# tsnuk/trade-AId-multimodal-transformer

Measured on AMD Instinct MI355X. Metric: training tokens/sec/GPU, 4-modality 1M-row synthetic, at 1/2/4/8 MI355X, higher is better.
Workload: dtype bf16; 1 GPU; C1: 4-modality 1M-row synthetic, d256 L6 T256 (BASELINE configs[1]); model=multimodal-transformer, global_batch=64, seq_len=256, n_embd=256, n_head=8, n_layer=6, modalities=4, parallelism=dp1

## Files before the change

### include/mmt.h

```cpp
#ifndef MMT_H_
#define MMT_H_
#include <stdint.h>

#ifdef __cplusplus
extern "C" {
#endif

#define MMT_MAX_MODALITIES 8

enum mmt_status {
  MMT_OK = 0,
  MMT_ERR_INVALID = -1,
  MMT_ERR_UNSUPPORTED = -2,
  MMT_ERR_HIP = -3,
  MMT_ERR_STATE = -4
};

typedef struct mmt_config {
  int32_t num_modalities;
  int32_t n_embd;
  int32_t n_head;
  int32_t n_layer;
  int32_t block_size;
  int32_t vocab_sizes[MMT_MAX_MODALITIES];
// ... 114 lines not shown
                   const int32_t* vocab, uint32_t* mt_state, const uint32_t* words, int64_t nwords, void* scratch,
                   int64_t scratch_bytes, int32_t* status);
int mmt_attn_set_ring(int v);
int mmt_attn_set_mask_g(int g);
int mmt_gemm_set_t2(int v);

int mmt_gemm_set_variant(int variant);
int mmt_op_gemm(void* stream, int32_t a_kc, int32_t b_kc, int32_t epi, int32_t splits, int32_t M, int32_t N,
                int32_t K, const void* A, int32_t lda, const void* B, int32_t ldb, const float* bias,
                const void* aux, int32_t ldaux, const float* resid, int32_t ldres, float* o32, int32_t ldc,
                void* o16, int32_t ldo16, float alpha);
int mmt_op_gemm_qkv(void* stream, int32_t M, int32_t N, int32_t K, const void* A, int32_t lda, const void* B,
                    int32_t ldb, const float* bias, void* h1, int32_t ldh1, const float* w2, int32_t hh, void* out,
                    int32_t ld_out);
int mmt_op_gemm_wgrad(void* stream, int32_t M, int32_t N, int32_t K, const void* A, int32_t lda, const void* B,
                      int32_t ldb, float* out, int32_t ldc, float alpha, void* slab, int64_t slab_bytes);
int mmt_op_mlp2(void* stream, int32_t M, int32_t C, const void* x, int32_t ldx, const void* w0, int32_t ldw0,
                const float* b0, const void* w2, int32_t ldw2, const float* b2, void* h, int32_t ldh, const float* resid,
                float* out, void* out16, uint32_t drop_key, uint32_t drop_thr, float drop_scale, const float* lnf_gamma,
                const float* lnf_beta, void* lnf_y, float* lnf_mean, float* lnf_rstd);
int mmt_op_mlp2_bwd(void* stream, int32_t M, int32_t C, const void* dy, int32_t lddy, const void* w2, int32_t ldw2,
                    const void* h, int32_t ldh, float alpha, const void* w0, int32_t ldw0, void* dh, int32_t lddh,
                    float* db0, void* dx);
int mmt_op_layernorm_fwd(void* stream, int32_t R, int32_t C, const float* x, const float* gamma, const float* beta,
                         void* y16, float* mean, float* rstd);
int mmt_op_layernorm_bwd(void* stream, int32_t R, int32_t C, const float* x, const float* gamma, const float* mean,
                         const float* rstd, const float* dy, float* dx, void* dx16, float* dgamma, float* dbeta);
int mmt_op_gemm_ln_bwd(void* stream, int32_t M, int32_t N, int32_t K, const void* A, int32_t lda, const void* B,
                       int32_t ldb, float alpha, const float* x, const float* gamma, const float* mean,
                       const float* rstd, float* dx, void* dx16, float* dgamma, float* dbeta, float* dsum,
                       uint32_t drop_key, uint32_t drop_thr, float drop_scale);
int mmt_op_attention_fwd(void* stream, int32_t B, int32_t T, int32_t H, int32_t hs, int32_t nstreams,
                         const void* q, int32_t q_ld, const void* const* k, const void* const* v, int32_t kv_ld,
                         int32_t kv_hstride, void* o, int32_t o_ld, void* const* oj, float* const* lse);
int mmt_op_attention_bwd(void* stream, int32_t B, int32_t T, int32_t H, int32_t hs, int32_t nstreams,
                         const void* q, int32_t q_ld, const void* const* k, const void* const* v, int32_t kv_ld,
                         int32_t kv_hstride, const void* o, int32_t o_ld, const void* const* oj,
                         const float* const* lse, const void* dout, int32_t dout_ld, float* const* dvec, void* dq,
                         int32_t dq_ld, void* const* dk, void* const* dv, int32_t dkv_ld, int32_t dkv_hstride);
int mmt_op_attention_bwd_ws(void* stream, int32_t B, int32_t T, int32_t H, int32_t hs, int32_t nstreams,
                            const void* q, int32_t q_ld, const void* const* k, const void* const* v, int32_t kv_ld,
                            int32_t kv_hstride, const void* o, int32_t o_ld, const void* const* oj,
                            const float* const* lse, const void* dout, int32_t dout_ld, float* const* dvec, void* dq,
                            int32_t dq_ld, void* const* dk, void* const* dv, int32_t dkv_ld, int32_t dkv_hstride,
                            float* dq32, int32_t dq32_ld);
int mmt_op_attention_fwd_h1(void* stream, int32_t B, int32_t T, int32_t H, const void* h1, int32_t ld_h1,
// ... 2 lines not shown
                            const float* w2, const void* o, int32_t o_ld, const float* lse, const void* dout,
                            int32_t dout_ld, void* dh1, float* dw2, float* db1);
int mmt_op_qkv2_fwd(void* stream, int32_t R, int32_t nblk, int32_t hs, const void* h1, int32_t ld_h1,
                    const float* w2, void* out, int32_t ld_out);
int mmt_op_qkv2_bwd(void* stream, int32_t R, int32_t nblk, int32_t hs, const void* h1, int32_t ld_h1,
                    const float* w2, const void* dout, int32_t ld_out, void* dh1, float* dw2);
int mmt_op_colsum(void* stream, int32_t R, int32_t N, const void* x, int32_t ld, float* out, float alpha);
int mmt_op_ordered_sum(void* stream, int32_t nparts, int32_t n, const float* parts, int64_t ld, float* dst);
int mmt_op_cross_entropy(void* stream, int32_t R, int32_t V, const float* logits, const int64_t* tgt,
                         void* dlogits, int32_t ld_d, float* loss);
int mmt_op_embedding_fwd(void* stream, int32_t B, int32_t T, int32_t C, int32_t V, const int64_t* idx,
                         const float* tok, const float* pos, float* x);
int mmt_op_embedding_bwd(void* stream, int32_t B, int32_t T, int32_t C, int32_t V, const int64_t* idx,
                         const float* dx, float* dtok, float* dpos);
int mmt_op_embedding_bwd_ws(void* stream, int32_t B, int32_t T, int32_t C, int32_t V, const int64_t* idx,
                            const float* dx, float* dtok, float* dpos, float* scratch);
int mmt_emb_set_sort(int on);
int mmt_qkv2_set_coal(int on);
int mmt_set_relu_bits(int on);
int mmt_set_drop_copy_fuse(int on);
int mmt_set_attn_qkv2(int on);
int mmt_set_attn_qkv_onchip(int bits);
int mmt_mlp2_set_bm(int bm);

int mmt_op_mx_quant(void* stream, int32_t rows, int32_t cols, const float* src, int32_t ld_src, void* dst8,
                    int32_t ld8, void* s8, int32_t lds8);
int mmt_op_gemm_f8(void* stream, int32_t epi, int32_t M, int32_t N, int32_t K, const void* A8, int32_t lda,
                   const void* sa, int32_t lds_a, const void* B8, int32_t ldb, const void* sb, int32_t lds_b,
                   const float* bias, const float* resid, int32_t ldres, float* o32, int32_t ldc, void* o16,
                   int32_t ldo16, void* o8, int32_t ld8, void* s8, int32_t lds8);
int mmt_op_layernorm_fwd_f8(void* stream, int32_t R, int32_t C, const float* x, const float* gamma, const float* beta,
                            void* y16, float* mean, float* rstd, void* y8, int32_t ld8, void* s8, int32_t lds8);

#ifdef __cplusplus
}
#endif
#endif
```

### trade-aid-multimodal-transformer_amd/csrc/mmt_engine.hip

```cpp
#include <hip/hip_runtime.h>

#include <algorithm>
#include <cmath>
#include <cstdio>
#include <cstdlib>
#include <cstring>
#include <string>
#include <vector>

#include "mmt.h"
#include "mmt_common.h"
#include "mmt_kernels.h"

namespace {

constexpr int MAXM = MMT_MAX_MODALITIES;

inline int64_t rup(int64_t x, int64_t a) { return (x + a - 1) / a * a; }
inline int r8(int x) { return (int)rup(x < 1 ? 1 : x, 8); }

struct Mat {
  int64_t off = -1;
  int rows = 0, cols = 0;
  int64_t pk = 0;
// ... 63 lines not shown

}

static int g_relu_bits = mmt_env_int("MMT_RELU_BITS", 0);
extern "C" int mmt_set_relu_bits(int on) {
  const int old = g_relu_bits;
  g_relu_bits = on;
  return old;
}
static int g_drop_copy_fuse = mmt_env_int("MMT_DROP_COPY_FUSE", 1);
extern "C" int mmt_set_drop_copy_fuse(int on) {
  const int old = g_drop_copy_fuse;
  g_drop_copy_fuse = on;
  return old;
}

static int g_attn_qkv2 = mmt_env_int("MMT_ATTN_QKV2", 1);
extern "C" int mmt_set_attn_qkv2(int on) {
  const int old = g_attn_qkv2;
  g_attn_qkv2 = on;
  return old;
}

static int g_attn_qkv_onchip = mmt_env_int("MMT_ATTN_QKV_ONCHIP", 3) & 3;
extern "C" int mmt_set_attn_qkv_onchip(int bits) {
  const int old = g_attn_qkv_onchip;
  g_attn_qkv_onchip = bits & 3;
  return old;
}

struct mmt_ctx {
  mmt_config cfg;
  int M, C, H, L, T, hs, hh;
  int V[MAXM];
  bool any_cross = false;
  int ncross = 0;
  std::vector<TensorInfo> tensors;
  std::vector<LM> lm;
  PostM post[MAXM];
  int64_t pos_off = 0;
  int64_t nparams = 0, nactive = 0;
  int64_t emb_begin = 0, emb_end = 0, post_begin = 0, post_end = 0;
  std::vector<int64_t> layer_begin, layer_end;
  std::vector<PackSeg> segs;
  std::vector<int> tasks;
  std::vector<MxSeg> mxsegs;
// ... 587 lines not shown
      Mlp2Batch& b = chunk[i / MMT_MLP2_GROUP];
      b.g1[b.count] = g1s[i];
      b.g2[b.count] = g2s[i];
      ++b.count;
    }
    for (int k = 0; k < nch; ++k)
      if (!(bwd ? mmt_mlp2_bwd_ok(chunk[k]) : mmt_mlp2_ok(chunk[k]))) return false;
    if (bwd)
      for (int k = 0; k < nch; ++k) det_arm(chunk[k]);
    const int id = probe_begin(what, s);
    for (int k = 0; k < nch; ++k) ok(bwd ? mmt_launch_mlp2_bwd(chunk[k], s) : mmt_launch_mlp2(chunk[k], s), what);
    if (id >= 0) {
      double fl = 0, by = 0;
      GemmBatch g1{}, g2{};
      g1.count = g2.count = n;
      for (int g = 0; g < n; ++g) { g1.p[g] = g1s[g]; g2.p[g] = g2s[g]; }
      gemm_cost(g1, bwd ? EPI_DTANH_BF16 : EPI_BIAS_TANH_BF16, &fl, &by);
      gemm_cost(g2, bwd ? EPI_STORE_BF16 : EPI_BIAS_RESID_F32, &fl, &by);
      for (int g = 0; g < n; ++g) by -= (double)g2s[g].M * g2s[g].K * 2.0;
      probe_end(id, s, fl, by);
    }
    return true;
  }
  bool gemm_resid_ln(const GemmBatch& b, const char* what) {
    if (rc != MMT_OK || !mmt_gemm_resid_ln_ok(b)) return false;
    const int id = probe_begin(what, s);
    ok(mmt_launch_gemm_resid_ln(b, s), what);
    if (id >= 0) {
      double fl = 0, by = 0;
      gemm_cost(b, EPI_BIAS_RESID_F32, &fl, &by);
      for (int g = 0; g < b.count; ++g)
        if (b.p[g].lnf_y) by += (double)b.p[g].M * b.p[g].N * 2.0 + b.p[g].M * 8.0;
      probe_end(id, s, fl, by);
    }
    return true;
  }
  int gemm_hint = 0;
  void gemm(const GemmBatch& b, bool akc, bool bkc, int epi, int splits, const char* what) {
    if (rc != MMT_OK) return;
    const int id = probe_begin(what, s);
    if (gemm_hint || det) {
      GemmBatch h = b;
      if (gemm_hint) h.tile_hint = gemm_hint;
      det_arm(h);
      ok(mmt_launch_gemm(h, akc, bkc, epi, splits, s), what);
    } else {
// ... 244 lines not shown
      ln2_done = fused && ln2_fuse;
      if (!fused) {
        for (int i = 0; i < M; ++i) g.p[i] = pg1[i];
        r.gemm(g, true, true, EPI_BIAS_TANH_BF16, 1, "proj0");
        for (int i = 0; i < M; ++i) { g.p[i] = pg2[i]; g.p[i].lnf_y = nullptr; }
        r.gemm(g, true, true, EPI_BIAS_RESID_F32, 1, "proj2");
      }
    }
    if (!ln2_done) {
      for (int i = 0; i < M; ++i) {
        lb.p[i].x = r.W<float>(a[i].x1); lb.p[i].gamma = r.P(x[i].ln2w); lb.p[i].beta = r.P(x[i].ln2b);
        lb.p[i].y = r.W<bf16_t>(a[i].c); lb.p[i].mean = r.W<float>(a[i].mean2); lb.p[i].rstd = r.W<float>(a[i].rstd2);
        ln8(lb.p[i], a[i].c8, a[i].cs8);
      }
      r.ok(mmt_launch_ln_fwd(lb, R, C, r.s), "ln2_fwd");
    }
    for (int i = 0; i < M; ++i) {
      g.p[i] = f8 ? gp_f8(r.W<uint8_t>(a[i].c8), C, r.W<uint8_t>(a[i].cs8), ldsC, w8, x[i].F0, R)
                  : gp_fwd(r.W<bf16_t>(a[i].c), C, wpk, x[i].F0, R);
      g.p[i].bias = r.P(x[i].bf0); g.p[i].o16 = r.W<bf16_t>(a[i].f); g.p[i].ldo16 = 4 * C;
      if (r.c->relu_bits) { g.p[i].mask8 = r.W<uint8_t>(a[i].fm); g.p[i].ldm8 = 4 * C / 8; }
      if (f8) { g.p[i].o8 = r.W<uint8_t>(a[i].f8); g.p[i].ld8 = 4 * C; g.p[i].s8 = r.W<uint8_t>(a[i].fs8); g.p[i].lds8 = ldsF; }
    }
    if (f8) r.gemm8(g, EPI_BIAS_RELU_BF16, "ffn0");
    else r.gemm(g, true, true, EPI_BIAS_RELU_BF16, 1, "ffn0");
    for (int i = 0; i < M; ++i) g.p[i].mask8 = nullptr;
    for (int i = 0; i < M; ++i) {
      g.p[i] = f8 ? gp_f8(r.W<uint8_t>(a[i].f8), 4 * C, r.W<uint8_t>(a[i].fs8), ldsF, w8, x[i].F2, R)
                  : gp_fwd(r.W<bf16_t>(a[i].f), 4 * C, wpk, x[i].F2, R);
      g.p[i].bias = r.P(x[i].bf2); g.p[i].resid = r.W<float>(a[i].x1); g.p[i].ldres = C;
      g.p[i].o32 = r.W<float>(a[i].x2); g.p[i].ldc = C;
      if (c->any_cross) { g.p[i].o16 = r.W<bf16_t>(a[i].x2h); g.p[i].ldo16 = C; }
      r.set_drop(g.p[i], l, i, DS_FFN);
    }
    bool lnc_done = false;
    if (fuse_fwd) {
      for (int i = 0; i < M; ++i) {
        GemmProblem& q = g.p[i];
        if (c->any_cross && x[i].cross) {
          q.lnf_gamma = r.P(x[i].lncw); q.lnf_beta = r.P(x[i].lncb); q.lnf_y = r.W<bf16_t>(a[i].d);
          q.lnf_mean = r.W<float>(a[i].meanc); q.lnf_rstd = r.W<float>(a[i].rstdc);
        } else if (l + 1 < c->L) {
          const LM& xn = c->lm[(size_t)(l + 1) * M + i];
          const ActLM& an = p.act[(size_t)(l + 1) * M + i];
          q.lnf_gamma = r.P(xn.ln1w); q.lnf_beta = r.P(xn.ln1b); q.lnf_y = r.W<bf16_t>(an.a);
          q.lnf_mean = r.W<float>(an.mean1); q.lnf_rstd = r.W<float>(an.rstd1);
        } else {
          q.lnf_gamma = r.P(c->post[i].lnw); q.lnf_beta = r.P(c->post[i].lnb); q.lnf_y = r.W<bf16_t>(p.lnf16[i]);
          q.lnf_mean = r.W<float>(p.meanf[i]); q.lnf_rstd = r.W<float>(p.rstdf[i]);
        }
      }
      if (r.gemm_resid_ln(g, "ffn2")) {
        for (int i = 0; i < M; ++i) {
          if (c->any_cross && x[i].cross) lnc_done = true;
          else if (l + 1 < c->L) ln1_done[i] = 1;
          else lnf_done[i] = 1;
        }
      } else {
        for (int i = 0; i < M; ++i) g.p[i].lnf_y = nullptr;
        r.gemm(g, true, true, EPI_BIAS_RESID_F32, 1, "ffn2");
      }
    } else if (f8) {
      r.gemm8(g, EPI_BIAS_RESID_F32, "ffn2");
    } else {
      r.gemm(g, true, true, EPI_BIAS_RESID_F32, 1, "ffn2");
    }
    for (int i = 0; i < M; ++i) g.p[i].lnf_y = nullptr;
    std::vector<const float*> xout(M);
    for (int i = 0; i < M; ++i) xout[i] = r.W<float>(a[i].x2);
    if (c->any_cross) {
      std::vector<int> cx;
      for (int i = 0; i < M; ++i) if (x[i].cross) cx.push_back(i);
      LnBatch lc{}; lc.count = (int)cx.size();
      GemmBatch gq{}; gq.count = (int)cx.size();
      for (size_t u = 0; u < cx.size(); ++u) {
        const int i = cx[u];
        lc.p[u].x = r.W<float>(a[i].x2); lc.p[u].gamma = r.P(x[i].lncw); lc.p[u].beta = r.P(x[i].lncb);
        lc.p[u].y = r.W<bf16_t>(a[i].d); lc.p[u].mean = r.W<float>(a[i].meanc); lc.p[u].rstd = r.W<float>(a[i].rstdc);
        ln8(lc.p[u], a[i].d8, a[i].ds8);
        gq.p[u] = f8 ? gp_f8(r.W<uint8_t>(a[i].d8), C, r.W<uint8_t>(a[i].ds8), ldsC, w8, x[i].Wq, R)
                     : gp_fwd(r.W<bf16_t>(a[i].d), C, wpk, x[i].Wq, R);
        gq.p[u].o16 = r.W<bf16_t>(a[i].qc); gq.p[u].ldo16 = C;
      }
      if (!lnc_done) r.ok(mmt_launch_ln_fwd(lc, R, C, r.s), "lnc_fwd");
      if (f8) r.gemm8(gq, EPI_STORE_BF16, "ca_q");
      else r.gemm(gq, true, true, EPI_STORE_BF16, 1, "ca_q");
      GemmBatch gk{}; gk.count = 0;
      for (int i : cx) {
// ... 1000 lines not shown
```

### trade-aid-multimodal-transformer_amd/csrc/mmt_gemm_dev.h

```cpp
#pragma once
#include "mmt_common.h"
#include "mmt_kernels.h"

#include <stdint.h>

template <int WM_, int WN_, int TM_, int TN_>
struct TileCfg {
  static constexpr int WM = WM_, WN = WN_, TM = TM_, TN = TN_;
  static constexpr int NW = WM * WN, NT = 64 * NW;
  static constexpr int BM = WM * TM * 32, BN = WN * TN * 32;
};
using TileS = TileCfg<2, 2, 2, 2>;
using TileL = TileCfg<2, 4, 4, 2>;
using TileW = TileCfg<1, 8, 4, 2>;

typedef __attribute__((address_space(3))) void lds_void;

__device__ __forceinline__ float* det_of(const GemmBatch& batch, int prob) {
  return batch.det.base ? batch.det.base + (int64_t)prob * batch.det.stride : nullptr;
}

template <int BK>
__device__ __forceinline__ int kc_swz(int chunk, int row) {
  return BK == 64 ? (chunk ^ ((row >> 1) & 7)) : (chunk ^ ((row >> 2) & 3));
// ... 152 lines not shown
  const int h = lane >> 5, r = lane & 31;
#pragma unroll
  for (int i = 0; i < TN; ++i)
#pragma unroll
    for (int j = 0; j < TM; ++j) {
      const int mf = wm * TM * 32 + 32 * j;
      if (mf / EPI_ROWS != pass) continue;
      const int ml = mf - pass * EPI_ROWS + r;
#pragma unroll
      for (int g = 0; g < 4; ++g) {
        const int nl = wn * TN * 32 + 32 * i + 8 * g + 4 * h;
        *reinterpret_cast<f32x4*>(ct + ml * CT + nl) =
            f32x4{acc[i][j][4 * g], acc[i][j][4 * g + 1], acc[i][j][4 * g + 2], acc[i][j][4 * g + 3]};
      }
    }
}
template <class TL, int EPI_ROWS>
__device__ __forceinline__ void stage_acc(f32x4 (&acc)[4][8], float* ct, int pass, int lane, int wave) {
  constexpr int CT = TL::BN + 4;
  const int wr = wave >> 2, wc = wave & 3;
#pragma unroll
  for (int mb = 0; mb < 8; ++mb) {
    const int mf = wr * 128 + 16 * mb;
    if (mf / EPI_ROWS != pass) continue;
    const int ml = mf - pass * EPI_ROWS + (lane & 15);
#pragma unroll
    for (int nb = 0; nb < 4; ++nb)
      *reinterpret_cast<f32x4*>(ct + ml * CT + wc * 64 + 16 * nb + 4 * (lane >> 4)) = acc[nb][mb];
  }
}

template <class TL, int EPI, int EPI_ROWS, bool PRE = false, class ACC>
__device__ __forceinline__ void epilogue_swap(const GemmProblem& P, ACC& acc, char* lds,
                                              float* o32, float alpha, int m0, int n0, int tid, int lane, int wave,
                                              float* det = nullptr) {
  constexpr int GBM = TL::BM, GBN = TL::BN, NW = TL::NW, NT = TL::NT, TM = TL::TM, TN = TL::TN;
  const int M = P.M, N = P.N;
  const int wm = wave / TL::WN, wn = wave % TL::WN;
  const int h = lane >> 5, r = lane & 31;
  constexpr int CT = GBN + 4;
  constexpr int TPR = GBN / 8;
  constexpr int RPI = NT / TPR;
  constexpr int IT = EPI_ROWS / RPI;
  float* ct = reinterpret_cast<float*>(lds);
  const int c8 = tid % TPR;
  const int rsub = tid / TPR;
// ... 381 lines not shown
```

### trade-aid-multimodal-transformer_amd/csrc/mmt_kernels.h

```cpp
#pragma once
#include <hip/hip_runtime.h>
#include <stdint.h>
#include "mmt_det.h"

#ifndef MMT_MAX_GROUP
#define MMT_MAX_GROUP 8
#endif
typedef uint16_t bf16_t;

enum MmtEpi {
  EPI_STORE_BF16 = 0,
  EPI_BIAS_TANH_BF16,
  EPI_BIAS_RELU_BF16,
  EPI_BIAS_RESID_F32,
  EPI_STORE_F32,
  EPI_DTANH_BF16,
  EPI_DRELU_BF16,
  EPI_ACC_F32,
  EPI_ATOMIC_F32,
  EPI_LN_BWD_F32,
  EPI_COUNT
};

struct GemmProblem {
// ... 45 lines not shown
  unsigned long long* stamps;
  DetScratch det;
};

hipError_t mmt_launch_gemm(const GemmBatch& b, bool a_kc, bool b_kc, int epi, int splits, hipStream_t s);
bool mmt_gemm_ln_bwd_ok(const GemmBatch& b);
bool mmt_gemm_resid_ln_ok(const GemmBatch& b);
hipError_t mmt_launch_gemm_resid_ln(const GemmBatch& b, hipStream_t s);
hipError_t mmt_launch_gemm_ln_bwd(const GemmBatch& b, hipStream_t s);
hipError_t mmt_launch_gemm_wgrad(const GemmBatch& b, float* slab, int64_t slab_bytes, hipStream_t s);

#define MMT_MLP2_GROUP 4
struct Mlp2Batch {
  GemmProblem g1[MMT_MLP2_GROUP];
  GemmProblem g2[MMT_MLP2_GROUP];
  int count;
  DetScratch det;
};
static_assert(sizeof(Mlp2Batch) <= 4096, "Mlp2Batch is a kernel argument");
bool mmt_mlp2_ok(const Mlp2Batch& b);
hipError_t mmt_launch_mlp2(const Mlp2Batch& b, hipStream_t s);
bool mmt_mlp2_bwd_ok(const Mlp2Batch& b);
hipError_t mmt_launch_mlp2_bwd(const Mlp2Batch& b, hipStream_t s);
hipError_t mmt_launch_gemm_f8(const GemmBatch& b, int epi, hipStream_t s);
bool mmt_gemm_wgrad_big(const GemmBatch& b);

struct LnProblem {
  const float* x;
  const float* gamma;
  const float* beta;
  bf16_t* y;
  float* mean;
  float* rstd;
  uint8_t* y8;
  uint8_t* s8;
  int ld8, lds8;
  const float* dy;
  float* dx;
  bf16_t* dx16;
  float* dgamma;
  float* dbeta;
  uint32_t drop_key, drop_thr;
  float drop_scale;
  float* dsum;
};
struct LnBatch {
// ... 166 lines not shown
```

### trade-aid-multimodal-transformer_amd/csrc/mmt_ops.hip

```cpp
#include <hip/hip_runtime.h>

#include "mmt.h"
#include "mmt_kernels.h"

static int st(hipError_t e) { return e == hipSuccess ? MMT_OK : MMT_ERR_HIP; }

extern "C" {

int mmt_op_gemm(void* stream, int32_t a_kc, int32_t b_kc, int32_t epi, int32_t splits, int32_t M, int32_t N,
                int32_t K, const void* A, int32_t lda, const void* B, int32_t ldb, const float* bias, const void* aux,
                int32_t ldaux, const float* resid, int32_t ldres, float* o32, int32_t ldc, void* o16, int32_t ldo16,
                float alpha) {
  if (epi < 0 || epi >= EPI_COUNT || M < 0 || N < 0 || K < 0) return MMT_ERR_INVALID;
  if ((lda & 7) || (ldb & 7)) return MMT_ERR_INVALID;
  GemmBatch b{};
  b.count = 1;
  GemmProblem& p = b.p[0];
  p.A = (const bf16_t*)A; p.lda = lda; p.B = (const bf16_t*)B; p.ldb = ldb; p.bias = bias;
  p.aux = (const bf16_t*)aux; p.ldaux = ldaux; p.resid = resid; p.ldres = ldres; p.o32 = o32; p.ldc = ldc;
  p.o16 = (bf16_t*)o16; p.ldo16 = ldo16; p.alpha = alpha; p.M = M; p.N = N; p.K = K;
  const hipError_t e = mmt_launch_gemm(b, a_kc != 0, b_kc != 0, epi, splits, (hipStream_t)stream);
  if (e == hipErrorInvalidValue) return MMT_ERR_UNSUPPORTED;
  return st(e);
}
// ... 25 lines not shown
  if (e == hipErrorInvalidValue) return MMT_ERR_UNSUPPORTED;
  return st(e);
}

int mmt_op_mlp2(void* stream, int32_t M, int32_t C, const void* x, int32_t ldx, const void* w0, int32_t ldw0,
                const float* b0, const void* w2, int32_t ldw2, const float* b2, void* h, int32_t ldh, const float* resid,
                float* out, void* out16, uint32_t drop_key, uint32_t drop_thr, float drop_scale, const float* lnf_gamma,
                const float* lnf_beta, void* lnf_y, float* lnf_mean, float* lnf_rstd) {
  if (M < 1 || C < 2) return MMT_ERR_INVALID;
  Mlp2Batch b{};
  b.count = 1;
  GemmProblem& p1 = b.g1[0];
  p1.A = (const bf16_t*)x; p1.lda = ldx; p1.B = (const bf16_t*)w0; p1.ldb = ldw0; p1.bias = b0;
  p1.o16 = (bf16_t*)h; p1.ldo16 = ldh; p1.alpha = 1.f; p1.M = M; p1.N = C / 2; p1.K = C;
  GemmProblem& p2 = b.g2[0];
  p2.A = (const bf16_t*)h; p2.lda = ldh; p2.B = (const bf16_t*)w2; p2.ldb = ldw2; p2.bias = b2;
  p2.resid = resid; p2.ldres = C; p2.o32 = out; p2.ldc = C; p2.o16 = (bf16_t*)out16; p2.ldo16 = C;
  p2.alpha = 1.f; p2.M = M; p2.N = C; p2.K = C / 2;
  p2.drop_key = drop_key; p2.drop_thr = drop_thr; p2.drop_scale = drop_scale;
  p2.lnf_gamma = lnf_gamma; p2.lnf_beta = lnf_beta; p2.lnf_y = (bf16_t*)lnf_y; p2.lnf_mean = lnf_mean;
  p2.lnf_rstd = lnf_rstd;
  if (!mmt_mlp2_ok(b)) return MMT_ERR_UNSUPPORTED;
  return st(mmt_launch_mlp2(b, (hipStream_t)stream));
}

int mmt_op_mlp2_bwd(void* stream, int32_t M, int32_t C, const void* dy, int32_t lddy, const void* w2, int32_t ldw2,
                    const void* h, int32_t ldh, float alpha, const void* w0, int32_t ldw0, void* dh, int32_t lddh,
                    float* db0, void* dx) {
  if (M < 1 || C < 2) return MMT_ERR_INVALID;
  Mlp2Batch b{};
  b.count = 1;
  GemmProblem& p1 = b.g1[0];
  p1.A = (const bf16_t*)dy; p1.lda = lddy; p1.B = (const bf16_t*)w2; p1.ldb = ldw2; p1.aux = (const bf16_t*)h;
  p1.ldaux = ldh; p1.o16 = (bf16_t*)dh; p1.ldo16 = lddh; p1.dbias = db0; p1.alpha = alpha; p1.M = M; p1.N = C / 2;
  p1.K = C;
  GemmProblem& p2 = b.g2[0];
  p2.A = (const bf16_t*)dh; p2.lda = lddh; p2.B = (const bf16_t*)w0; p2.ldb = ldw0; p2.o16 = (bf16_t*)dx; p2.ldo16 = C;
  p2.alpha = 1.f; p2.M = M; p2.N = C; p2.K = C / 2;
  if (!mmt_mlp2_bwd_ok(b)) return MMT_ERR_UNSUPPORTED;
  return st(mmt_launch_mlp2_bwd(b, (hipStream_t)stream));
}

int mmt_op_layernorm_fwd(void* stream, int32_t R, int32_t C, const float* x, const float* gamma, const float* beta,
                         void* y16, float* mean, float* rstd) {
  LnBatch b{};
  b.count = 1;
// ... 233 lines not shown
```

### trade-aid-multimodal-transformer_amd/mmt_build.py

```python
import concurrent.futures as cf
import os
import subprocess
import sys

HERE = os.path.dirname(os.path.abspath(__file__))
REPO = os.path.dirname(HERE)
CSRC = os.path.join(HERE, "csrc")
OBJ = os.path.join(CSRC, "build")
LIB = os.path.join(HERE, "libmmt_hip.so")
HIPCC = os.environ.get("HIPCC", "/opt/rocm/bin/hipcc")
SOURCES = ["mmt_gemm.hip", "mmt_gemm8.hip", "mmt_mlp2.hip", "mmt_attn.hip", "mmt_attn_oc.hip", "mmt_attn2.hip", "mmt_elem.hip", "mmt_stats.hip", "mmt_qkv2.hip", "mmt_engine.hip", "mmt_ops.hip", "mmt_batch.hip", "mmt_decode.hip"]
FLAGS = ["--offload-arch=gfx950", "-O3", "-std=c++17", "-fPIC", "-I" + os.path.join(REPO, "include"), "-I" + CSRC,
         "-Wall", "-Wno-unused-function", "-Wno-unused-variable", "-Wno-unused-result"]

VGPR_FORM = ["-mllvm", "-amdgpu-mfma-vgpr-form=1"]
FILE_FLAGS = {"mmt_attn.hip": ["-fno-slp-vectorize"] + VGPR_FORM, "mmt_attn_oc.hip": ["-fno-slp-vectorize"] + VGPR_FORM,
              "mmt_attn2.hip": ["-fno-slp-vectorize"],
              "mmt_qkv2.hip": VGPR_FORM}


def _deps_mtime():
    hdrs = [os.path.join(CSRC, f) for f in os.listdir(CSRC) if f.endswith(".h")]
    hdrs.append(os.path.join(REPO, "include", "mmt.h"))
    return max(os.path.getmtime(h) for h in hdrs)


def _compile(src, force):
    s = os.path.join(CSRC, src)
    o = os.path.join(OBJ, src.replace(".hip", ".o"))
    if not force and os.path.exists(o) and os.path.getmtime(o) >= max(os.path.getmtime(s), _deps_mtime()):
        return o
    cmd = [HIPCC] + FLAGS + FILE_FLAGS.get(src, []) + ["-c", s, "-o", o]
    r = subprocess.run(cmd, capture_output=True, text=True)
    if r.returncode != 0:
# ... 23 lines not shown
```

### trade-aid-multimodal-transformer_amd/mmt_lib.py

```python
import ctypes
import os

import torch

HERE = os.path.dirname(os.path.abspath(__file__))
LIB_PATH = os.environ.get("MMT_LIB_PATH") or os.path.join(HERE, "libmmt_hip.so")
MAX_MOD = 8

c_i32 = ctypes.c_int32
c_i64 = ctypes.c_int64
c_f32 = ctypes.c_float
c_vp = ctypes.c_void_p
c_cp = ctypes.c_char_p


class MmtConfig(ctypes.Structure):
    _fields_ = [
        ("num_modalities", c_i32),
        ("n_embd", c_i32),
        ("n_head", c_i32),
        ("n_layer", c_i32),
        ("block_size", c_i32),
        ("vocab_sizes", c_i32 * MAX_MOD),
        ("cross_attention", c_i32 * MAX_MOD),
# ... 91 lines not shown
    "mmt_set_deterministic": (c_i32, [c_vp, c_i32]),
    "mmt_get_deterministic": (c_i32, [c_vp]),
    "mmt_probe_count": (c_i32, [c_vp]),
    "mmt_probe_read_at": (c_i32, [c_vp, c_i32, ctypes.POINTER(ctypes.c_double), ctypes.POINTER(c_i64),
                                  ctypes.POINTER(ctypes.c_double), ctypes.POINTER(ctypes.c_double)]),
    "mmt_batch_jitter":(c_i32, [c_vp, c_vp, c_i64, c_i32, c_i32, ctypes.c_uint64, ctypes.c_uint64]),
    "mmt_batch_indices": (c_i32, [c_vp, c_i32, c_vp, c_vp, c_i32, c_i32, ctypes.c_uint64, ctypes.c_uint64, c_vp]),
    "mmt_batch_gather": (c_i32, [c_vp, c_i32, ctypes.POINTER(c_vp), c_vp, c_i32, c_i32, ctypes.POINTER(c_vp),
                                 ctypes.POINTER(c_vp)]),
    "mmt_exact_words_bytes": (c_i64, [c_i64]),
    "mmt_exact_walk_scratch_bytes": (c_i64, [c_i64, c_i64]),
    "mmt_exact_gen": (c_i32, [c_vp, c_vp, c_vp, c_i64]),
    "mmt_exact_walk": (c_i32, [c_vp, c_i32, ctypes.POINTER(c_vp), ctypes.POINTER(c_i64), ctypes.POINTER(c_i32),
                               ctypes.POINTER(c_i32), c_vp, c_vp, c_i64, c_vp, c_i64, c_vp]),
    "mmt_attn_set_ring": (c_i32, [ctypes.c_int]),
    "mmt_attn_set_mask_g": (c_i32, [ctypes.c_int]),
    "mmt_gemm_set_t2": (c_i32, [ctypes.c_int]),
    "mmt_emb_set_sort": (c_i32, [ctypes.c_int]),
    "mmt_set_relu_bits": (c_i32, [ctypes.c_int]),
    "mmt_set_drop_copy_fuse": (c_i32, [ctypes.c_int]),
    "mmt_set_attn_qkv2": (c_i32, [ctypes.c_int]),
    "mmt_set_attn_qkv_onchip": (c_i32, [ctypes.c_int]),
    "mmt_mlp2_set_bm": (c_i32, [ctypes.c_int]),
    "mmt_qkv2_set_coal": (c_i32, [ctypes.c_int]),
    "mmt_gemm_set_variant": (c_i32, [ctypes.c_int]),
    "mmt_op_gemm": (c_i32, [c_vp, c_i32, c_i32, c_i32, c_i32, c_i32, c_i32, c_i32, c_vp, c_i32, c_vp, c_i32, c_vp,
                            c_vp, c_i32, c_vp, c_i32, c_vp, c_i32, c_vp, c_i32, c_f32]),
    "mmt_op_gemm_qkv": (c_i32, [c_vp, c_i32, c_i32, c_i32, c_vp, c_i32, c_vp, c_i32, c_vp, c_vp, c_i32, c_vp, c_i32,
                                c_vp, c_i32]),
    "mmt_op_gemm_wgrad": (c_i32, [c_vp, c_i32, c_i32, c_i32, c_vp, c_i32, c_vp, c_i32, c_vp, c_i32, c_f32, c_vp, c_i64]),
    "mmt_op_gemm_ln_bwd": (c_i32, [c_vp, c_i32, c_i32, c_i32, c_vp, c_i32, c_vp, c_i32, c_f32, c_vp, c_vp, c_vp, c_vp,
                                   c_vp, c_vp, c_vp, c_vp, c_vp, ctypes.c_uint32, ctypes.c_uint32, c_f32]),
    "mmt_op_mlp2": (c_i32, [c_vp, c_i32, c_i32, c_vp, c_i32, c_vp, c_i32, c_vp, c_vp, c_i32, c_vp, c_vp, c_i32, c_vp,
                            c_vp, c_vp, ctypes.c_uint32, ctypes.c_uint32, c_f32, c_vp, c_vp, c_vp, c_vp, c_vp]),
    "mmt_op_mlp2_bwd": (c_i32, [c_vp, c_i32, c_i32, c_vp, c_i32, c_vp, c_i32, c_vp, c_i32, c_f32, c_vp, c_i32, c_vp,
                                c_i32, c_vp, c_vp]),
    "mmt_op_layernorm_fwd": (c_i32, [c_vp, c_i32, c_i32, c_vp, c_vp, c_vp, c_vp, c_vp, c_vp]),
    "mmt_op_layernorm_bwd": (c_i32, [c_vp, c_i32, c_i32, c_vp, c_vp, c_vp, c_vp, c_vp, c_vp, c_vp, c_vp, c_vp]),
    "mmt_op_attention_fwd": (c_i32, [c_vp, c_i32, c_i32, c_i32, c_i32, c_i32, c_vp, c_i32, ctypes.POINTER(c_vp),
                                     ctypes.POINTER(c_vp), c_i32, c_i32, c_vp, c_i32, ctypes.POINTER(c_vp),
                                     ctypes.POINTER(c_vp)]),
    "mmt_op_attention_bwd": (c_i32, [c_vp, c_i32, c_i32, c_i32, c_i32, c_i32, c_vp, c_i32, ctypes.POINTER(c_vp),
                                     ctypes.POINTER(c_vp), c_i32, c_i32, c_vp, c_i32, ctypes.POINTER(c_vp),
                                     ctypes.POINTER(c_vp), c_vp, c_i32, ctypes.POINTER(c_vp), c_vp, c_i32,
                                     ctypes.POINTER(c_vp), ctypes.POINTER(c_vp), c_i32, c_i32]),
    "mmt_op_attention_bwd_ws": (c_i32, [c_vp, c_i32, c_i32, c_i32, c_i32, c_i32, c_vp, c_i32, ctypes.POINTER(c_vp),
                                        ctypes.POINTER(c_vp), c_i32, c_i32, c_vp, c_i32, ctypes.POINTER(c_vp),
                                        ctypes.POINTER(c_vp), c_vp, c_i32, ctypes.POINTER(c_vp), c_vp, c_i32,
                                        ctypes.POINTER(c_vp), ctypes.POINTER(c_vp), c_i32, c_i32, c_vp, c_i32]),
    "mmt_op_attention_fwd_h1": (c_i32, [c_vp, c_i32, c_i32, c_i32, c_vp, c_i32, c_vp, c_vp, c_i32, c_vp]),
    "mmt_op_attention_bwd_h1": (c_i32, [c_vp, c_i32, c_i32, c_i32, c_vp, c_i32, c_vp, c_vp, c_i32, c_vp, c_vp, c_i32,
                                        c_vp, c_vp, c_vp]),
    "mmt_op_qkv2_fwd": (c_i32, [c_vp, c_i32, c_i32, c_i32, c_vp, c_i32, c_vp, c_vp, c_i32]),
    "mmt_op_qkv2_bwd": (c_i32, [c_vp, c_i32, c_i32, c_i32, c_vp, c_i32, c_vp, c_vp, c_i32, c_vp, c_vp]),
    "mmt_op_colsum": (c_i32, [c_vp, c_i32, c_i32, c_vp, c_i32, c_vp, c_f32]),
    "mmt_op_ordered_sum": (c_i32, [c_vp, c_i32, c_i32, c_vp, c_i64, c_vp]),
    "mmt_op_cross_entropy": (c_i32, [c_vp, c_i32, c_i32, c_vp, c_vp, c_vp, c_i32, c_vp]),
# ... 58 lines not shown
```

Measured before the change: 8.579 million tokens/s.

## Fuse FFN up-projection and down-projection into one on-chip forward kernel

```diff
diff --git a/include/mmt.h b/include/mmt.h
--- a/include/mmt.h
+++ b/include/mmt.h
@@ -160,6 +160,11 @@
 int mmt_op_mlp2_bwd(void* stream, int32_t M, int32_t C, const void* dy, int32_t lddy, const void* w2, int32_t ldw2,
                     const void* h, int32_t ldh, float alpha, const void* w0, int32_t ldw0, void* dh, int32_t lddh,
                     float* db0, void* dx);
+int mmt_op_ffn(void* stream, int32_t count, const int32_t* M, int32_t C, const void* const* x, int32_t ldx,
+               const void* w0, int32_t ldw0, const float* b0, const void* w2, int32_t ldw2, const float* b2,
+               void* const* h, int32_t ldh, const float* const* resid, float* const* out, void* const* out16,
+               uint32_t drop_key, uint32_t drop_thr, float drop_scale, const float* lnf_gamma, const float* lnf_beta,
+               void* const* lnf_y, float* const* lnf_mean, float* const* lnf_rstd);
 int mmt_op_layernorm_fwd(void* stream, int32_t R, int32_t C, const float* x, const float* gamma, const float* beta,
                          void* y16, float* mean, float* rstd);
 int mmt_op_layernorm_bwd(void* stream, int32_t R, int32_t C, const float* x, const float* gamma, const float* mean,
@@ -208,6 +213,7 @@
 int mmt_set_attn_qkv2(int on);
 int mmt_set_attn_qkv_onchip(int bits);
 int mmt_mlp2_set_bm(int bm);
+int mmt_set_ffn_fused(int on);
 
 int mmt_op_mx_quant(void* stream, int32_t rows, int32_t cols, const float* src, int32_t ld_src, void* dst8,
                     int32_t ld8, void* s8, int32_t lds8);
diff --git a/trade-aid-multimodal-transformer_amd/csrc/mmt_engine.hip b/trade-aid-multimodal-transformer_amd/csrc/mmt_engine.hip
--- a/trade-aid-multimodal-transformer_amd/csrc/mmt_engine.hip
+++ b/trade-aid-multimodal-transformer_amd/csrc/mmt_engine.hip
@@ -109,6 +109,12 @@
   return old;
 }
 
+static int g_ffn_fused = mmt_env_int("MMT_FFN_FUSED", 1);
+extern "C" int mmt_set_ffn_fused(int on) {
+  const int old = g_ffn_fused;
+  g_ffn_fused = on;
+  return old;
+}
 static int g_attn_qkv_onchip = mmt_env_int("MMT_ATTN_QKV_ONCHIP", 3) & 3;
 extern "C" int mmt_set_attn_qkv_onchip(int bits) {
   const int old = g_attn_qkv_onchip;
@@ -742,6 +748,32 @@
     }
     return true;
   }
+  bool ffn(const GemmProblem* g1s, const GemmProblem* g2s, int n, const char* what) {
+    if (rc != MMT_OK || n < 1) return false;
+    Mlp2Batch chunk[(MMT_MAX_GROUP + MMT_MLP2_GROUP - 1) / MMT_MLP2_GROUP] = {};
+    const int nch = (n + MMT_MLP2_GROUP - 1) / MMT_MLP2_GROUP;
+    for (int i = 0; i < n; ++i) {
+      Mlp2Batch& b = chunk[i / MMT_MLP2_GROUP];
+      b.g1[b.count] = g1s[i];
+      b.g2[b.count] = g2s[i];
+      ++b.count;
+    }
+    for (int k = 0; k < nch; ++k)
+      if (!mmt_ffn_ok(chunk[k])) return false;
+    const int id = probe_begin(what, s);
+    for (int k = 0; k < nch; ++k) ok(mmt_launch_ffn(chunk[k], s), what);
+    if (id >= 0) {
+      double fl = 0, by = 0;
+      GemmBatch g1{}, g2{};
+      g1.count = g2.count = n;
+      for (int g = 0; g < n; ++g) { g1.p[g] = g1s[g]; g2.p[g] = g2s[g]; }
+      gemm_cost(g1, EPI_BIAS_RELU_BF16, &fl, &by);
+      gemm_cost(g2, EPI_BIAS_RESID_F32, &fl, &by);
+      for (int g = 0; g < n; ++g) by -= (double)g2s[g].M * g2s[g].K * 2.0;
+      probe_end(id, s, fl, by);
+    }
+    return true;
+  }
   bool gemm_resid_ln(const GemmBatch& b, const char* what) {
     if (rc != MMT_OK || !mmt_gemm_resid_ln_ok(b)) return false;
     const int id = probe_begin(what, s);
@@ -1032,8 +1064,11 @@
       if (r.c->relu_bits) { g.p[i].mask8 = r.W<uint8_t>(a[i].fm); g.p[i].ldm8 = 4 * C / 8; }
       if (f8) { g.p[i].o8 = r.W<uint8_t>(a[i].f8); g.p[i].ld8 = 4 * C; g.p[i].s8 = r.W<uint8_t>(a[i].fs8); g.p[i].lds8 = ldsF; }
     }
-    if (f8) r.gemm8(g, EPI_BIAS_RELU_BF16, "ffn0");
-    else r.gemm(g, true, true, EPI_BIAS_RELU_BF16, 1, "ffn0");
+    const GemmBatch gf0 = g;
+    auto run_ffn0 = [&] {
+      if (f8) r.gemm8(gf0, EPI_BIAS_RELU_BF16, "ffn0");
+      else r.gemm(gf0, true, true, EPI_BIAS_RELU_BF16, 1, "ffn0");
+    };
     for (int i = 0; i < M; ++i) g.p[i].mask8 = nullptr;
     for (int i = 0; i < M; ++i) {
       g.p[i] = f8 ? gp_f8(r.W<uint8_t>(a[i].f8), 4 * C, r.W<uint8_t>(a[i].fs8), ldsF, w8, x[i].F2, R)
@@ -1060,7 +1095,11 @@
           q.lnf_mean = r.W<float>(p.meanf[i]); q.lnf_rstd = r.W<float>(p.rstdf[i]);
         }
       }
-      if (r.gemm_resid_ln(g, "ffn2")) {
+    }
+    const bool ffn_one = !f8 && !c->relu_bits && C == 256 && g_ffn_fused != 0 && r.ffn(gf0.p, g.p, M, "ffn");
+    if (!ffn_one) run_ffn0();
+    if (fuse_fwd) {
+      if (ffn_one || r.gemm_resid_ln(g, "ffn2")) {
         for (int i = 0; i < M; ++i) {
           if (c->any_cross && x[i].cross) lnc_done = true;
           else if (l + 1 < c->L) ln1_done[i] = 1;
@@ -1070,10 +1109,9 @@
         for (int i = 0; i < M; ++i) g.p[i].lnf_y = nullptr;
         r.gemm(g, true, true, EPI_BIAS_RESID_F32, 1, "ffn2");
       }
-    } else if (f8) {
-      r.gemm8(g, EPI_BIAS_RESID_F32, "ffn2");
-    } else {
-      r.gemm(g, true, true, EPI_BIAS_RESID_F32, 1, "ffn2");
+    } else if (!ffn_one) {
+      if (f8) r.gemm8(g, EPI_BIAS_RESID_F32, "ffn2");
+      else r.gemm(g, true, true, EPI_BIAS_RESID_F32, 1, "ffn2");
     }
     for (int i = 0; i < M; ++i) g.p[i].lnf_y = nullptr;
     std::vector<const float*> xout(M);
diff --git a/trade-aid-multimodal-transformer_amd/csrc/mmt_ffn.hip b/trade-aid-multimodal-transformer_amd/csrc/mmt_ffn.hip
--- /dev/null
+++ b/trade-aid-multimodal-transformer_amd/csrc/mmt_ffn.hip
@@ -0,0 +1,249 @@
+#include "mmt_gemm_dev.h"
+
+#include <algorithm>
+#include <type_traits>
+
+namespace {
+
+constexpr int FFN_BM = 128;
+constexpr int FFN_C = 256;
+constexpr int FFN_HID = 1024;
+constexpr int FFN_CH = 128;
+constexpr int FFN_NCH = FFN_HID / FFN_CH;
+constexpr int FFN_SLOT = 16384;
+constexpr int FFN_DSLOT = 2 * FFN_SLOT;
+constexpr int FFN_NS = 3;
+constexpr int FFN_RING = FFN_NS * FFN_DSLOT;
+constexpr int FFN_NSTEP = FFN_NCH * 4;
+constexpr int FFN_HPITCH = FFN_CH * 2;
+constexpr int FFN_HIMG = FFN_BM * FFN_HPITCH;
+constexpr int FFN_LDS = FFN_RING + FFN_HIMG + FFN_HID * 4;
+constexpr int FFN_EPI_ROWS = 32;
+using FfnT2 = TileCfg<2, 4, 2, 2>;
+static_assert(FFN_EPI_ROWS * (FfnT2::BN + 4) * 4 <= FFN_RING, "the epilogue's staging tile reuses the ring");
+static_assert(FFN_BM * FFN_C * 2 <= (FFN_NS - 1) * FFN_DSLOT, "the x tile is staged in ring slots 1..2");
+static_assert(FFN_LDS <= 160 * 1024, "LDS per workgroup");
+
+__device__ __forceinline__ int h_off(int m, int chunk) { return m * FFN_HPITCH + ((chunk ^ (m & 15)) << 4); }
+
+__device__ __forceinline__ f32x4 mfma16(bf16x8 a, bf16x8 b, f32x4 c) {
+  return __builtin_amdgcn_mfma_f32_16x16x32_bf16(a, b, c, 0, 0, 0);
+}
+
+__device__ __forceinline__ void store16(const i32x4& rsrc, int voff, u32x4 v) {
+  asm volatile("buffer_store_dwordx4 %0, %1, %2, 0 offen\n\ts_nop 1" : : "v"(v), "v"(voff), "s"(rsrc) : "memory");
+}
+
+constexpr int ffn_wait(int c, int d) {
+  const int i = 4 * c + d;
+  int n = i + 1 < FFN_NSTEP ? 4 : 0;
+  for (int j = i - 2; j < i; ++j)
+    if (j >= 0 && (j & 3) >= 2) n += 2;
+  return n;
+}
+
+}
+
+__global__ __launch_bounds__(512, 1) void ffn_fwd_kernel(Mlp2Batch batch) {
+  constexpr int NW = 8;
+  __shared__ __attribute__((aligned(1024))) char lds[FFN_LDS];
+  char* const himg = lds + FFN_RING;
+  float* const b0s = reinterpret_cast<float*>(himg + FFN_HIMG);
+
+  const int prob = blockIdx.z;
+  const GemmProblem& P1 = batch.g1[prob];
+  const GemmProblem& P2 = batch.g2[prob];
+  const int M = __builtin_amdgcn_readfirstlane(P1.M);
+  const int ntiles = (M + FFN_BM - 1) / FFN_BM;
+  const int tile = xcd_tile(blockIdx.x, gridDim.x);
+  if (tile >= ntiles) return;
+  const int m0 = tile * FFN_BM;
+  const int tid = threadIdx.x, lane = tid & 63;
+  const int wave = __builtin_amdgcn_readfirstlane(tid >> 6);
+  const int wm = wave >> 2, wn = wave & 3;
+  const int wm1 = wave >> 1, wn1 = wave & 1;
+  const int h = lane >> 5, r = lane & 31;
+  const int g16 = lane >> 4, l16 = lane & 15;
+
+  const int ldx = __builtin_amdgcn_readfirstlane(P1.lda), ldw0 = __builtin_amdgcn_readfirstlane(P1.ldb);
+  const int ldw2 = __builtin_amdgcn_readfirstlane(P2.ldb), ldh = __builtin_amdgcn_readfirstlane(P1.ldo16);
+  const bf16_t* const W0p = sgpr_ptr(P1.B);
+  const i32x4 rx = op_rsrc<true>(P1.A, ldx, M, FFN_C, m0, 0);
+  const i32x4 rw2 = op_rsrc<true>(P2.B, ldw2, FFN_C, FFN_HID, 0, 0);
+  const i32x4 rh = make_rsrc(reinterpret_cast<const char*>(P1.o16) + (int64_t)m0 * ldh * 2, (int64_t)(M - m0) * ldh * 2);
+
+  auto issue = [&](int slot, int c, auto DC) {
+    constexpr int D = decltype(DC)::value;
+    char* st = lds + slot * FFN_DSLOT;
+    if constexpr (D < 2) {
+      const i32x4 rw0 = op_rsrc<true>(W0p, ldw0, FFN_HID, FFN_C, c * FFN_CH, 0);
+      issue_tile<64, true, FFN_CH, NW>(rw0, st, ldw0, FFN_HID, FFN_C, c * FFN_CH, 128 * D, wave, lane);
+      issue_tile<64, true, FFN_CH, NW>(rw0, st + FFN_SLOT, ldw0, FFN_HID, FFN_C, c * FFN_CH, 128 * D + 64, wave, lane);
+    } else {
+      issue_tile<32, true, FFN_C, NW>(rw2, st, ldw2, FFN_C, FFN_HID, 0, c * FFN_CH + 64 * (D - 2), wave, lane);
+      issue_tile<32, true, FFN_C, NW>(rw2, st + FFN_SLOT, ldw2, FFN_C, FFN_HID, 0, c * FFN_CH + 64 * (D - 2) + 32, wave, lane);
+    }
+  };
+
+  char* const xst = lds + FFN_DSLOT;
+#pragma unroll
+  for (int t = 0; t < 4; ++t) issue_tile<64, true, FFN_BM, NW>(rx, xst + t * 16384, ldx, M, FFN_C, m0, 64 * t, wave, lane);
+  issue(0, 0, std::integral_constant<int, 0>{});
+  {
+    const float2 bv = *reinterpret_cast<const float2*>(P1.bias + 2 * tid);
+    *reinterpret_cast<float2*>(b0s + 2 * tid) = bv;
+  }
+  wait_vm(0);
+  asm volatile("s_waitcnt lgkmcnt(0)" ::: "memory");
+  __builtin_amdgcn_s_barrier();
+  bf16x8 xr[16];
+#pragma unroll
+  for (int t = 0; t < 4; ++t)
+#pragma unroll
+    for (int s = 0; s < 4; ++s) xr[4 * t + s] = frag<64, true, FFN_BM>(xst + t * 16384, wm1 * 32, s, lane);
+  asm volatile("s_waitcnt lgkmcnt(0)" ::: "memory");
+  __builtin_amdgcn_s_barrier();
+  issue(1, 0, std::integral_constant<int, 1>{});
+
+  f32x16 acc1[2];
+  f32x4 acc2[4][4];
+#pragma unroll
+  for (int i = 0; i < 4; ++i)
+#pragma unroll
+    for (int j = 0; j < 4; ++j) acc2[i][j] = f32x4{0.f, 0.f, 0.f, 0.f};
+
+  auto step = [&](int c, int slot, auto DC, auto KC) {
+    constexpr int D = decltype(DC)::value;
+    constexpr int KIND = decltype(KC)::value;
+    constexpr int CREP = KIND == 0 ? 0 : KIND == 1 ? 1 : FFN_NCH - 1;
+    static_assert(ffn_wait(1, D) == ffn_wait(FFN_NCH - 2, D), "steady-state counts");
+    wait_vm(ffn_wait(CREP, D));
+    asm volatile("s_waitcnt lgkmcnt(0)" ::: "memory");
+    __builtin_amdgcn_s_barrier();
+    u32x4 hv[2];
+    int hvoff[2];
+    if constexpr (D >= 2) {
+#pragma unroll
+      for (int u = 0; u < 2; ++u) {
+        const int idx = (2 * (D - 2) + u) * 512 + tid;
+        const int m = idx >> 4, cc = idx & 15;
+        hv[u] = *reinterpret_cast<const u32x4*>(himg + h_off(m, cc));
+        hvoff[u] = m0 + m < M ? (m * ldh + c * FFN_CH + 8 * cc) * 2 : 0x7fffffff;
+      }
+    }
+    const int nslot = slot == 0 ? FFN_NS - 1 : slot - 1;
+    if constexpr (D < 2) issue(nslot, c, std::integral_constant<int, D + 2>{});
+    else if constexpr (KIND != 2) issue(nslot, c + 1, std::integral_constant<int, D - 2>{});
+    if constexpr (D >= 2) {
+      store16(rh, hvoff[0], hv[0]);
+      store16(rh, hvoff[1], hv[1]);
+    }
+    if constexpr (D < 2) {
+      if constexpr (D == 0) {
+#pragma unroll
+        for (int i = 0; i < 2; ++i)
+#pragma unroll
+          for (int e = 0; e < 16; ++e) acc1[i][e] = 0.f;
+      }
+#pragma unroll
+      for (int q = 0; q < 2; ++q) {
+        const char* imgW = lds + slot * FFN_DSLOT + q * FFN_SLOT;
+#pragma unroll
+        for (int s = 0; s < 4; ++s) {
+          bf16x8 fb[2];
+#pragma unroll
+          for (int i = 0; i < 2; ++i) fb[i] = frag<64, true, FFN_CH>(imgW, wn1 * 64 + 32 * i, s, lane);
+#pragma unroll
+          for (int i = 0; i < 2; ++i) acc1[i] = mfma32(fb[i], xr[8 * D + 4 * q + s], acc1[i]);
+        }
+      }
+      if constexpr (D == 1) {
+        const int m = wm1 * 32 + r;
+#pragma unroll
+        for (int i = 0; i < 2; ++i)
+#pragma unroll
+          for (int g = 0; g < 4; ++g) {
+            const f32x4 bv = *reinterpret_cast<const f32x4*>(b0s + c * FFN_CH + wn1 * 64 + 32 * i + 8 * g + 4 * h);
+            const uint32_t lo = pack2bf(fmaxf(acc1[i][4 * g] + bv[0], 0.0f), fmaxf(acc1[i][4 * g + 1] + bv[1], 0.0f));
+            const uint32_t hi = pack2bf(fmaxf(acc1[i][4 * g + 2] + bv[2], 0.0f), fmaxf(acc1[i][4 * g + 3] + bv[3], 0.0f));
+            *reinterpret_cast<u32x2*>(himg + h_off(m, wn1 * 8 + 4 * i + g) + 8 * h) = u32x2{lo, hi};
+          }
+      }
+    } else {
+#pragma unroll
+      for (int q = 0; q < 2; ++q) {
+        const char* imgW = lds + slot * FFN_DSLOT + q * FFN_SLOT;
+        bf16x8 xf[4], wf[4];
+#pragma unroll
+        for (int mb = 0; mb < 4; ++mb)
+          xf[mb] = *reinterpret_cast<const bf16x8*>(himg + h_off(wm * 64 + 16 * mb + l16, 4 * (2 * (D - 2) + q) + g16));
+#pragma unroll
+        for (int nb = 0; nb < 4; ++nb) {
+          const int row = wn * 64 + 16 * nb + l16;
+          wf[nb] = *reinterpret_cast<const bf16x8*>(imgW + row * 64 + kc_swz<32>(g16, row) * 16);
+        }
+#pragma unroll
+        for (int nb = 0; nb < 4; ++nb)
+#pragma unroll
+          for (int mb = 0; mb < 4; ++mb) acc2[nb][mb] = mfma16(wf[nb], xf[mb], acc2[nb][mb]);
+      }
+    }
+  };
+
+  int slot = 0;
+  auto chunk = [&](int c, auto KC) {
+    auto next = [&] { slot = slot == FFN_NS - 1 ? 0 : slot + 1; };
+    step(c, slot, std::integral_constant<int, 0>{}, KC); next();
+    step(c, slot, std::integral_constant<int, 1>{}, KC); next();
+    step(c, slot, std::integral_constant<int, 2>{}, KC); next();
+    step(c, slot, std::integral_constant<int, 3>{}, KC); next();
+  };
+  chunk(0, std::integral_constant<int, 0>{});
+#pragma unroll 1
+  for (int c = 1; c < FFN_NCH - 1; ++c) chunk(c, std::integral_constant<int, 1>{});
+  chunk(FFN_NCH - 1, std::integral_constant<int, 2>{});
+
+  epilogue_swap<FfnT2, EPI_BIAS_RESID_F32, FFN_EPI_ROWS>(P2, acc2, lds, P2.o32, P2.alpha, m0, 0, tid, lane, wave);
+}
+
+static bool ffn_unused_clear(const GemmProblem& p1, const GemmProblem& p2) {
+  for (const GemmProblem* p : {&p1, &p2})
+    if (p->o8 || p->s8 || p->mask8 || p->qkv2_out || p->qkv2_h1_only || p->split_stride || p->sa || p->sb ||
+        p->ln_dgamma || p->ln_dbeta || p->ln_gamma || p->aux || p->dbias || p->alpha_ptr)
+      return false;
+  return !p1.resid && !p1.o32 && !p1.drop_thr && !p1.lnf_y && !p1.lnf_gamma && !p1.lnf_beta && !p1.lnf_mean &&
+         !p1.lnf_rstd;
+}
+
+bool mmt_ffn_ok(const Mlp2Batch& b) {
+  if (b.count <= 0 || b.count > MMT_MLP2_GROUP) return false;
+  for (int g = 0; g < b.count; ++g) {
+    const GemmProblem& p1 = b.g1[g];
+    const GemmProblem& p2 = b.g2[g];
+    if (p1.N != FFN_HID || p1.K != FFN_C || p2.N != FFN_C || p2.K != FFN_HID || p2.M != p1.M || p1.M < 1) return false;
+    if (!p1.A || !p1.B || !p1.bias || !p1.o16 || !p2.B || !p2.bias || !p2.resid || !p2.o32) return false;
+    if (p2.A != p1.o16 || p2.lda != p1.ldo16) return false;
+    if ((p1.lda & 7) || (p1.ldb & 7) || (p2.ldb & 7) || (p1.ldo16 & 7) || (p2.ldc & 3) || (p2.ldres & 3) ||
+        (p2.o16 && ((p2.ldo16 & 7) || p2.ldo16 < FFN_C)) || p1.lda < FFN_C || p1.ldb < FFN_C || p2.ldb < FFN_HID ||
+        p1.ldo16 < FFN_HID || p2.ldc < FFN_C || p2.ldres < FFN_C)
+      return false;
+    if (((uintptr_t)p1.A | (uintptr_t)p1.B | (uintptr_t)p2.B | (uintptr_t)p1.o16 | (uintptr_t)p2.o32 |
+         (uintptr_t)p2.resid | (uintptr_t)p1.bias | (uintptr_t)p2.bias | (uintptr_t)p2.o16) & 15)
+      return false;
+    if (!ffn_unused_clear(p1, p2)) return false;
+    if (p1.alpha != 1.0f || p2.alpha != 1.0f) return false;
+    if ((int64_t)513 * std::max(std::max(p1.lda, p1.ldb), std::max(p2.ldb, p1.ldo16)) * 2 >= ((int64_t)1 << 31)) return false;
+    const bool any = p2.lnf_y || p2.lnf_gamma || p2.lnf_beta || p2.lnf_mean || p2.lnf_rstd;
+    const bool all = p2.lnf_y && p2.lnf_gamma && p2.lnf_beta && p2.lnf_mean && p2.lnf_rstd;
+    if (any && (!all || (((uintptr_t)p2.lnf_y | (uintptr_t)p2.lnf_gamma | (uintptr_t)p2.lnf_beta) & 15))) return false;
+  }
+  return true;
+}
+
+hipError_t mmt_launch_ffn(const Mlp2Batch& b, hipStream_t s) {
+  if (!mmt_ffn_ok(b)) return hipErrorInvalidValue;
+  int mt = 0;
+  for (int g = 0; g < b.count; ++g) mt = std::max(mt, (b.g1[g].M + FFN_BM - 1) / FFN_BM);
+  hipLaunchKernelGGL(ffn_fwd_kernel, dim3(mt, 1, b.count), dim3(512), 0, s, b);
+  return hipGetLastError();
+}
diff --git a/trade-aid-multimodal-transformer_amd/csrc/mmt_gemm_dev.h b/trade-aid-multimodal-transformer_amd/csrc/mmt_gemm_dev.h
--- a/trade-aid-multimodal-transformer_amd/csrc/mmt_gemm_dev.h
+++ b/trade-aid-multimodal-transformer_amd/csrc/mmt_gemm_dev.h
@@ -198,6 +198,20 @@
 #pragma unroll
   for (int mb = 0; mb < 8; ++mb) {
     const int mf = wr * 128 + 16 * mb;
+    if (mf / EPI_ROWS != pass) continue;
+    const int ml = mf - pass * EPI_ROWS + (lane & 15);
+#pragma unroll
+    for (int nb = 0; nb < 4; ++nb)
+      *reinterpret_cast<f32x4*>(ct + ml * CT + wc * 64 + 16 * nb + 4 * (lane >> 4)) = acc[nb][mb];
+  }
+}
+template <class TL, int EPI_ROWS>
+__device__ __forceinline__ void stage_acc(f32x4 (&acc)[4][4], float* ct, int pass, int lane, int wave) {
+  constexpr int CT = TL::BN + 4;
+  const int wr = wave >> 2, wc = wave & 3;
+#pragma unroll
+  for (int mb = 0; mb < 4; ++mb) {
+    const int mf = wr * 64 + 16 * mb;
     if (mf / EPI_ROWS != pass) continue;
     const int ml = mf - pass * EPI_ROWS + (lane & 15);
 #pragma unroll
diff --git a/trade-aid-multimodal-transformer_amd/csrc/mmt_kernels.h b/trade-aid-multimodal-transformer_amd/csrc/mmt_kernels.h
--- a/trade-aid-multimodal-transformer_amd/csrc/mmt_kernels.h
+++ b/trade-aid-multimodal-transformer_amd/csrc/mmt_kernels.h
@@ -91,6 +91,8 @@
 hipError_t mmt_launch_mlp2(const Mlp2Batch& b, hipStream_t s);
 bool mmt_mlp2_bwd_ok(const Mlp2Batch& b);
 hipError_t mmt_launch_mlp2_bwd(const Mlp2Batch& b, hipStream_t s);
+bool mmt_ffn_ok(const Mlp2Batch& b);
+hipError_t mmt_launch_ffn(const Mlp2Batch& b, hipStream_t s);
 hipError_t mmt_launch_gemm_f8(const GemmBatch& b, int epi, hipStream_t s);
 bool mmt_gemm_wgrad_big(const GemmBatch& b);
 
diff --git a/trade-aid-multimodal-transformer_amd/csrc/mmt_ops.hip b/trade-aid-multimodal-transformer_amd/csrc/mmt_ops.hip
--- a/trade-aid-multimodal-transformer_amd/csrc/mmt_ops.hip
+++ b/trade-aid-multimodal-transformer_amd/csrc/mmt_ops.hip
@@ -71,6 +71,33 @@
   p2.lnf_rstd = lnf_rstd;
   if (!mmt_mlp2_ok(b)) return MMT_ERR_UNSUPPORTED;
   return st(mmt_launch_mlp2(b, (hipStream_t)stream));
+}
+
+int mmt_op_ffn(void* stream, int32_t count, const int32_t* M, int32_t C, const void* const* x, int32_t ldx,
+               const void* w0, int32_t ldw0, const float* b0, const void* w2, int32_t ldw2, const float* b2,
+               void* const* h, int32_t ldh, const float* const* resid, float* const* out, void* const* out16,
+               uint32_t drop_key, uint32_t drop_thr, float drop_scale, const float* lnf_gamma, const float* lnf_beta,
+               void* const* lnf_y, float* const* lnf_mean, float* const* lnf_rstd) {
+  if (count < 1 || !M || !x || !h || !resid || !out || C < 2) return MMT_ERR_INVALID;
+  if (count > MMT_MLP2_GROUP || C != 256) return MMT_ERR_UNSUPPORTED;
+  Mlp2Batch b{};
+  b.count = count;
+  for (int g = 0; g < count; ++g) {
+    if (M[g] < 1) return MMT_ERR_INVALID;
+    GemmProblem& p1 = b.g1[g];
+    p1.A = (const bf16_t*)x[g]; p1.lda = ldx; p1.B = (const bf16_t*)w0; p1.ldb = ldw0; p1.bias = b0;
+    p1.o16 = (bf16_t*)h[g]; p1.ldo16 = ldh; p1.alpha = 1.f; p1.M = M[g]; p1.N = 4 * C; p1.K = C;
+    GemmProblem& p2 = b.g2[g];
+    p2.A = (const bf16_t*)h[g]; p2.lda = ldh; p2.B = (const bf16_t*)w2; p2.ldb = ldw2; p2.bias = b2;
+    p2.resid = resid[g]; p2.ldres = C; p2.o32 = out[g]; p2.ldc = C;
+    p2.o16 = out16 ? (bf16_t*)out16[g] : nullptr; p2.ldo16 = C;
+    p2.alpha = 1.f; p2.M = M[g]; p2.N = C; p2.K = 4 * C;
+    p2.drop_key = drop_key; p2.drop_thr = drop_thr; p2.drop_scale = drop_scale;
+    p2.lnf_gamma = lnf_gamma; p2.lnf_beta = lnf_beta; p2.lnf_y = lnf_y ? (bf16_t*)lnf_y[g] : nullptr;
+    p2.lnf_mean = lnf_mean ? lnf_mean[g] : nullptr; p2.lnf_rstd = lnf_rstd ? lnf_rstd[g] : nullptr;
+  }
+  if (!mmt_ffn_ok(b)) return MMT_ERR_UNSUPPORTED;
+  return st(mmt_launch_ffn(b, (hipStream_t)stream));
 }
 
 int mmt_op_mlp2_bwd(void* stream, int32_t M, int32_t C, const void* dy, int32_t lddy, const void* w2, int32_t ldw2,
diff --git a/trade-aid-multimodal-transformer_amd/mmt_build.py b/trade-aid-multimodal-transformer_amd/mmt_build.py
--- a/trade-aid-multimodal-transformer_amd/mmt_build.py
+++ b/trade-aid-multimodal-transformer_amd/mmt_build.py
@@ -9,7 +9,7 @@
 OBJ = os.path.join(CSRC, "build")
 LIB = os.path.join(HERE, "libmmt_hip.so")
 HIPCC = os.environ.get("HIPCC", "/opt/rocm/bin/hipcc")
-SOURCES = ["mmt_gemm.hip", "mmt_gemm8.hip", "mmt_mlp2.hip", "mmt_attn.hip", "mmt_attn_oc.hip", "mmt_attn2.hip", "mmt_elem.hip", "mmt_stats.hip", "mmt_qkv2.hip", "mmt_engine.hip", "mmt_ops.hip", "mmt_batch.hip", "mmt_decode.hip"]
+SOURCES = ["mmt_gemm.hip", "mmt_gemm8.hip", "mmt_mlp2.hip", "mmt_ffn.hip", "mmt_attn.hip", "mmt_attn_oc.hip", "mmt_attn2.hip", "mmt_elem.hip", "mmt_stats.hip", "mmt_qkv2.hip", "mmt_engine.hip", "mmt_ops.hip", "mmt_batch.hip", "mmt_decode.hip"]
 FLAGS = ["--offload-arch=gfx950", "-O3", "-std=c++17", "-fPIC", "-I" + os.path.join(REPO, "include"), "-I" + CSRC,
          "-Wall", "-Wno-unused-function", "-Wno-unused-variable", "-Wno-unused-result"]
 
diff --git a/trade-aid-multimodal-transformer_amd/mmt_lib.py b/trade-aid-multimodal-transformer_amd/mmt_lib.py
--- a/trade-aid-multimodal-transformer_amd/mmt_lib.py
+++ b/trade-aid-multimodal-transformer_amd/mmt_lib.py
@@ -137,6 +137,7 @@
     "mmt_set_attn_qkv2": (c_i32, [ctypes.c_int]),
     "mmt_set_attn_qkv_onchip": (c_i32, [ctypes.c_int]),
     "mmt_mlp2_set_bm": (c_i32, [ctypes.c_int]),
+    "mmt_set_ffn_fused": (c_i32, [ctypes.c_int]),
     "mmt_qkv2_set_coal": (c_i32, [ctypes.c_int]),
     "mmt_gemm_set_variant": (c_i32, [ctypes.c_int]),
     "mmt_op_gemm": (c_i32, [c_vp, c_i32, c_i32, c_i32, c_i32, c_i32, c_i32, c_i32, c_vp, c_i32, c_vp, c_i32, c_vp,
@@ -148,6 +149,10 @@
                                    c_vp, c_vp, c_vp, c_vp, c_vp, ctypes.c_uint32, ctypes.c_uint32, c_f32]),
     "mmt_op_mlp2": (c_i32, [c_vp, c_i32, c_i32, c_vp, c_i32, c_vp, c_i32, c_vp, c_vp, c_i32, c_vp, c_vp, c_i32, c_vp,
                             c_vp, c_vp, ctypes.c_uint32, ctypes.c_uint32, c_f32, c_vp, c_vp, c_vp, c_vp, c_vp]),
+    "mmt_op_ffn": (c_i32, [c_vp, c_i32, ctypes.POINTER(c_i32), c_i32, ctypes.POINTER(c_vp), c_i32, c_vp, c_i32, c_vp,
+                           c_vp, c_i32, c_vp, ctypes.POINTER(c_vp), c_i32, ctypes.POINTER(c_vp), ctypes.POINTER(c_vp),
+                           ctypes.POINTER(c_vp), ctypes.c_uint32, ctypes.c_uint32, c_f32, c_vp, c_vp,
+                           ctypes.POINTER(c_vp), ctypes.POINTER(c_vp), ctypes.POINTER(c_vp)]),
     "mmt_op_mlp2_bwd": (c_i32, [c_vp, c_i32, c_i32, c_vp, c_i32, c_vp, c_i32, c_vp, c_i32, c_f32, c_vp, c_i32, c_vp,
                                 c_i32, c_vp, c_vp]),
     "mmt_op_layernorm_fwd": (c_i32, [c_vp, c_i32, c_i32, c_vp, c_vp, c_vp, c_vp, c_vp, c_vp]),
```

New measurement: 8.682 million tokens/s, median of 6. 1.01x the previous value.
